# arkCyber/whisper-rust

Hardware: AMD Instinct MI355X
Metric: real-time factor (audio-sec/wall-sec), greedy, 30 s synthetic chunks (higher is better)
Workload: dtype f16 operands / f32 accumulate; 1 GPU; ggml-small-shaped synthetic F16 model, greedy best_of=1 temperature_inc=0, 1 x 30 s 16 kHz f32 chunk per GPU, PCM resident in HBM; flash_attn=False, parallelism=chunk-dp1

## Files before the change

### whisper-rust_amd/csrc/wa_mega.hip

```cpp
#include "wa_device.h"
#include "wa_mega.h"

typedef unsigned long long u64;
#define GAS __attribute__((address_space(1)))
typedef GAS u64 gu64;
typedef GAS unsigned gu32;
typedef const GAS wa_f16 * gch;
typedef const GAS float * gcf;
typedef _Float16 half4v __attribute__((ext_vector_type(4)));
typedef unsigned u32x2 __attribute__((ext_vector_type(2)));
typedef unsigned u32x4 __attribute__((ext_vector_type(4)));

typedef const __attribute__((address_space(4))) wa_mega_args * mg_kargs;
__device__ __forceinline__ mg_kargs mg_uniform(mg_kargs p) {
    const unsigned long long v = (unsigned long long) p;
    const unsigned lo = __builtin_amdgcn_readfirstlane((unsigned) v), hi = __builtin_amdgcn_readfirstlane((unsigned) (v >> 32));
    return (mg_kargs) (((unsigned long long) hi << 32) | lo);
}

#define MG_THREADS 512
#define MG_NW (MG_THREADS / 64)
#define MG_NP3 4
#define MG_SPIN_LIMIT 20000u
#ifndef MG_DEFER
// ... 1054 lines not shown
#pragma unroll
        for (int cc = 0; cc < 32; ++cc) dv[cc] = (cc < 16 ? dbl0 : dbl1)[(cc & 15) * 64 + tid];
        __builtin_amdgcn_sched_barrier(0);
#pragma unroll
        for (int cc = 0; cc < 32; ++cc) sumf += dv[cc];
        if (tslot >= 0) mg_trace(A, tid == 0, tslot + 2, mg_now() + (sumf == 1e300 ? 1u : 0u));
        if constexpr (Q) {
            const float y = (float) sumf;
            float a = fabsf(y);
            a = fmaxf(a, dpp_f32<0x128>(a)); a = fmaxf(a, dpp_f32<0x124>(a)); a = fmaxf(a, dpp_f32<0x122>(a)); a = fmaxf(a, dpp_f32<0x121>(a));
            a = fmaxf(a, __shfl_xor(a, 16, 32));
            const float dsc = a / 127.f, id = a != 0.0f ? 127.f / a : 0.0f;
            const unsigned q = (unsigned) (int) rintf(y * id) & 0xffu;
            const unsigned w = q | (dpp_u32<0x101>(q) << 8) | (dpp_u32<0x102>(q) << 16) | (dpp_u32<0x103>(q) << 24);
            gu64 * eb = edge + (size_t) (2 * h + (tid >> 5)) * 9;
            if ((tid & 3) == 0) gr_store(eb + ((tid & 31) >> 2), seq, w);
            if ((tid & 31) == 0) gr_store(eb + 8, seq, __float_as_uint(h2f(f2h(dsc))));
        } else {
        const unsigned hv = (unsigned) f2h((float) sumf);
        const unsigned hi = dpp_u32<0x101>(hv);
        if ((tid & 1) == 0) gr_store(edge + ((h * 64 + tid) >> 1), seq, (hv & 0xffffu) | (hi << 16));
        }
    }
}

template <bool Q = false>
__device__ __forceinline__ void mg_role_self(mg_kargs A_, int idx_) {
    extern __shared__ __attribute__((aligned(16))) unsigned char smem[];
    const mg_kargs A = mg_uniform(A_);
    const int tid = threadIdx.x, lane = tid & 63;
    const int wave = __builtin_amdgcn_readfirstlane(tid >> 6);
    const int h = __builtin_amdgcn_readfirstlane(idx_);
    mg_ctl c; c.status = (gu32 *) A->status; c.seq = A->seq; c.dead = false;
    mg_chaos_start(c.seq);

    wa_f16 * Ks = (wa_f16 *) smem;
    wa_f16 * Vs = Ks + WA_MEGA_MAX_KV * 64;
    const mg_att_smem M = mg_att_carve(smem + (size_t) WA_MEGA_MAX_KV * 64 * 2 * 2, WA_MEGA_MAX_KV);
    const int d = A->d, n_kv = A->n_kv, kv_head = A->kv_head, L = A->n_layer;
    const int a = tid & 3, kslot = tid >> 2;
    if (wave == 0) mg_pick(A, lane, (int *) (smem + MG_PICK_OFF));
    for (int l = 0; l < L; ++l) {
        {
            const gch kc = (gch) A->kv_k + (size_t) l * A->kv_layer_stride + h * 64;
            const gch vc = (gch) A->kv_v + (size_t) l * A->kv_layer_stride + h * 64;
            const int n16 = n_kv * 8;
            u32x4 tk[8], tv[8];
#pragma unroll
            for (int j = 0; j < 8; ++j) {
                const int idx = tid + MG_THREADS * j;
                if (idx < n16) {
                    tk[j] = *(const GAS u32x4 *) (kc + (size_t) (idx >> 3) * d + (idx & 7) * 8);
                    tv[j] = *(const GAS u32x4 *) (vc + (size_t) (idx >> 3) * d + (idx & 7) * 8);
                }
            }
#pragma unroll
            for (int j = 0; j < 8; ++j) {
                const int idx = tid + MG_THREADS * j;
                if (idx < n16) { *(u32x4 *) (Ks + (size_t) idx * 8) = tk[j]; *(u32x4 *) (Vs + (size_t) idx * 8) = tv[j]; }
            }
        }
        mg_barrier();
        if (wave == 0) {
            unsigned v[2];
            const unsigned sp = mg_sweep<2>(mg_edge(A, l, E_QKV), [&](int k) {
                if (k == 0) return (lane < 32 ? 0 : (d >> 1)) + h * 32 + (lane & 31);
                return lane < 32 ? d + h * 32 + lane : -1; }, c, lane, v, 1000u + l);
            mg_trace(A, h == 0 && lane == 0, (l * 8 + 6) * 8 + 0, mg_now()); mg_trace(A, h == 0 && lane == 0, (l * 8 + 6) * 8 + 1, sp);
            if (lane < 32) { ((unsigned *) M.qs)[lane] = v[0]; ((unsigned *) (Vs + (size_t) kv_head * 64))[lane] = v[1]; }
            else ((unsigned *) (Ks + (size_t) kv_head * 64))[lane - 32] = v[0];
        }
        mg_barrier();
        float lmax = -INFINITY;
        {
            float qa[8], qb[8];
#pragma unroll
            for (int i = 0; i < 8; ++i) { qa[i] = h2f(M.qs[8 * a + i]); qb[i] = h2f(M.qs[32 + 8 * a + i]); }
            for (int c0 = 0; c0 < n_kv; c0 += MG_THREADS / 4) {
                const int cc = c0 + kslot, cl = cc < n_kv ? cc : n_kv - 1;
                const u32x4 ka = *(const u32x4 *) (Ks + (size_t) cl * 64 + 8 * a), kb = *(const u32x4 *) (Ks + (size_t) cl * 64 + 32 + 8 * a);
                const float r = mg_score(ka, kb, qa, qb, 1.0f);
                if (cc < n_kv) { if (a == 0) M.sc[cc] = r; lmax = fmaxf(lmax, r); }
            }
        }
        mg_trace(A, h == 0 && tid == 0, (l * 8 + 6) * 8 + 4, mg_now());
        {
            lmax = wave_max(lmax);
            if (lane == 0) M.red[wave] = lmax;
            mg_barrier();
            float mx = M.red[0];
#pragma unroll
            for (int k = 1; k < MG_NW; ++k) mx = fmaxf(mx, M.red[k]);
            const int n8 = n_kv & ~7, ng = n8 >> 3;
            float e = 0.0f;
            double ps = 0.0;
            if (tid < n_kv) e = tid < n8 ? wa_expf(M.sc[tid] - mx) : wa_expf_libm(M.sc[tid] - mx);
            {
                float t = e + dpp_f32<0x104>(e);
                t = t + dpp_f32<0x102>(t);
                t = t + dpp_f32<0x101>(t);
                if (tid < n8) ps = (tid & 7) == 0 ? (double) t : 0.0;
                else if (tid < n_kv) ps = (double) e;
            }
            ps = wave_sum_d(ps);
            if (lane == 0) M.redd[wave] = ps;
            mg_barrier();
            const double tot = ((M.redd[0] + M.redd[1]) + (M.redd[2] + M.redd[3])) + ((M.redd[4] + M.redd[5]) + (M.redd[6] + M.redd[7]));
            const double delta = (double) (ng + 8 + 16) * 0x1p-53 * tot * 1.000001;
            const float ilo = (float) (1.0 / (tot + delta)), ihi = (float) (1.0 / (tot - delta));
            if (ilo != ihi && tid == 0 && !c.dead) __hip_atomic_store(c.status, (unsigned) WA_MEGA_REDO, __ATOMIC_RELAXED, __HIP_MEMORY_SCOPE_AGENT);
            if (tid < n_kv) M.p16[tid] = f2h(e * ilo);
            mg_barrier();
        }
        mg_trace(A, h == 0 && tid == 0, (l * 8 + 6) * 8 + 5, mg_now());
        MG_CHAOS_ID(1000 + h, 21u, c.seq);
        const int np = n_kv & ~31, nsteps = np >> 5;
        {
            float acc[4] = { 0.0f, 0.0f, 0.0f, 0.0f };
            const int r0 = wave * 4;
            for (int s = 0; s < nsteps; ++s) {
#pragma unroll
                for (int i = 0; i < 4; ++i)
                    acc[i] = fmaf(h2f(Vs[(size_t) (s * 32 + r0 + i) * 64 + lane]), h2f(M.p16[s * 32 + r0 + i]), acc[i]);
            }
#pragma unroll
            for (int i = 0; i < 4; ++i) M.part[(r0 + i) * 64 + lane] = acc[i];
        }
        mg_barrier();
        mg_attn_finish<Q>(M.part, Vs + (size_t) np * 64, M.p16, np, n_kv - np, mg_edge(A, l, E_AO), h, c.seq, tid, (double *) (Ks + WA_MEGA_KV_ROOM * 64),
                          (double *) (Vs + WA_MEGA_KV_ROOM * 64), A, A->dbg && h == 0 && l == MG_WGTRACE_LAYER ? 3004 : -1);
        mg_trace(A, h == 0 && tid == 0, (l * 8 + 6) * 8 + 3, mg_now());
        mg_barrier();
    }
    unsigned pf[96];
    bool have_pf = false;
    float gw[MG_NP3], gb[MG_NP3];
    if (wave >= 1) mg_prefetch_logits<0, Q>(A, pf, have_pf, lane, wave);
    mg_ln_params<MG_NP3>(gw, gb, A->lnf_w, A->lnf_b, A->d, mg_slot(wave, MG_EX_FINAL), lane);
    mg_final<MG_NP3, 0, Q>(A, c, smem, pf, have_pf, gw, gb, lane, wave);
}

#define MG_CSTEPS 48
#define MG_CGR 2048
#define MG_CGR_MAX 0
#define MG_CGR_SUM 8
#define MG_CGR_XCC 16
#define MG_CGR_PART 64
#define MG_CX_XF 32768
#define MG_CX_XIN (MG_CX_XF + WA_MEGA_MAX_D * 4)
#define MG_CX_LNRED (MG_CX_XIN + WA_MEGA_MAX_D * 2)
#define MG_CX_END (MG_CX_LNRED + 256)
#define MG_CX_TRACE 6144

template <bool Q = false, int CQ = -1>
__device__ __forceinline__ void mg_role_cross(mg_kargs A_, int idx_) {
    extern __shared__ __attribute__((aligned(16))) unsigned char smem[];
    const mg_kargs A = mg_uniform(A_);
    int tid = threadIdx.x, lane = tid & 63;
    const int wave = __builtin_amdgcn_readfirstlane(tid >> 6);
    const int H = A->n_head;
    const int ci = __builtin_amdgcn_readfirstlane(idx_);
    const int h = ci >> 2, w = ci & 3;
    mg_ctl c; c.status = (gu32 *) A->status; c.seq = A->seq; c.dead = false;
    mg_chaos_start(c.seq);
    const unsigned seq = c.seq;

    float  * part  = (float *) smem;
    wa_f16 * vleft = (wa_f16 *) (smem + 8192);
    float  * sc    = (float *) (smem + 8192 + 4096);
    wa_f16 * p16   = (wa_f16 *) (smem + 8192 + 4096 + 1536);
    wa_f16 * pleft = (wa_f16 *) (smem + 8192 + 4096 + 1536 + 768);
    wa_f16 * qs    = (wa_f16 *) (smem + 8192 + 4096 + 1536 + 768 + 64);
    double * redd  = (double *) (smem + 8192 + 4096 + 1536 + 768 + 64 + 128);
    float  * red   = (float *) (smem + 8192 + 4096 + 1536 + 768 + 64 + 128 + 64);
    float  * bc    = red + 8;

    const int T = A->T, tpad = A->cross_tpad, L = A->n_layer;
    const float kq_scale = A->kq_scale;
    int a = tid & 3, ks = tid >> 2;
    const int np = T & ~31, nsteps = np >> 5, nl = T - np, n8 = T & ~7, ng = n8 >> 3;
    if (wave == 0) mg_pick(A, lane, (int *) (smem + MG_PICK_OFF));
    if (wave == 0) {
        const unsigned xcc = (unsigned) __builtin_amdgcn_s_getreg(20 | (3 << 11)) & 0xfu;
        gu64 * X0 = (gu64 *) A->cross_gr + (size_t) h * MG_CGR + MG_CGR_XCC;
        if (lane == 0) gr_store(X0 + w, seq, xcc);
        unsigned v[1];
        mg_sweep<1>(X0, [&](int) { return lane < 4 ? lane : -1; }, c, lane, v, 2900u);
        const bool same = lane >= 4 || v[0] == xcc;
        if (lane == 0) bc[2] = __builtin_amdgcn_ballot_w64(same) == ~0ull && !c.dead ? 1.0f : 0.0f;
    }
    mg_barrier();
    const bool local = bc[2] != 0.0f;
    const __attribute__((address_space(4))) wa_mega_layer * Ly = (const __attribute__((address_space(4))) wa_mega_layer *) A->layers;
    float  * xf    = (float *) (smem + MG_CX_XF);
    wa_f16 * xin   = (wa_f16 *) (smem + MG_CX_XIN);
    double * lnred = (double *) (smem + MG_CX_LNRED);
    const int d = A->d;
    for (int l = 0; l < L; ++l) {
        if constexpr (CQ >= 0) {
            unsigned z = threadIdx.x; asm volatile("" : "+v"(z));
            tid = (int) z; lane = tid & 63; a = tid & 3; ks = tid >> 2;
        }
        gu64 * X = (gu64 *) A->cross_gr + ((size_t) l * H + h) * MG_CGR;
        const gch kp = (gch) A->cross_k + (size_t) l * A->cross_layer_stride + (size_t) h * tpad * 64;
        const gch vp = (gch) A->cross_v + (size_t) l * A->cross_layer_stride + (size_t) h * tpad * 64;
        u32x4 ka[3], kb[3];
        unsigned short vv[MG_CSTEPS];
#pragma unroll
        for (int p = 0; p < 3; ++p) {
            const int o = p * 128 + ks, cc = 32 * (o >> 3) + 8 * w + (o & 7);
            if (cc < T) { ka[p] = *(const GAS u32x4 *) (kp + (size_t) cc * 64 + 8 * a); kb[p] = *(const GAS u32x4 *) (kp + (size_t) cc * 64 + 32 + 8 * a); }
        }
#pragma unroll
        for (int s = 0; s < MG_CSTEPS; ++s) if (s < nsteps) vv[s] = *(const GAS unsigned short *) (vp + (size_t) (32 * s + 8 * w + wave) * 64 + lane);
        if (w == 0 && tid < 256) {
            const int row = tid >> 3;
            if (row < nl) *(u32x4 *) (vleft + (size_t) tid * 8) = *(const GAS u32x4 *) (vp + (size_t) (np + row) * 64 + (tid & 7) * 8);
        }
        if constexpr (CQ >= 0) {
            unsigned pf[96];
            float gw[2], gb[2];
            const int row = 64 * h + 8 * wave + (lane >> 3);
            const gch wrow = (gch) Ly[l].cq_w + (size_t) row * d + 4 * (lane & 7);
            mg_pf8<CQ>(pf, wrow, true, d >> 5, 0);
            const float bias = ((gcf) Ly[l].cq_b)[row];
            mg_ln_params<2>(gw, gb, Ly[l].ln2_w, Ly[l].ln2_b, d, mg_slot(wave, 0u), lane);
            mg_trace(A, ci == 0 && lane == 0 && wave == 0, (l * 8 + 7) * 8 + 2, mg_now());
            mg_ln3<2>(A, c, mg_edge(A, l, E_X1), gw, gb, mg_slot(wave, 0u), lane, xf, xin, lnred, 2000u + l,
                      ci == 0 && wave == 0 ? MG_CX_TRACE + l * 8 : -1);
            MG_CHAOS_ID(2000 + ci, 30u, seq);
            float v = mg_dot8<CQ>(pf, wrow, true, d >> 5, xin, lane & 7, true);
            v = v + bias;
            const unsigned hq = (unsigned) f2h(v);
            if ((lane & 7) == 0) qs[8 * wave + (lane >> 3)] = (wa_f16) hq;
            if (A->dbg && w == 0) mg_pub_h2(mg_edge(A, l, E_QC), seq, true, row, hq, lane);
            mg_trace(A, ci == 0 && lane == 0 && wave == 0, (l * 8 + 7) * 8 + 0, mg_now());
            if (A->dbg && l == MG_WGTRACE_LAYER && w == 0) mg_trace(A, tid == 0, 3200 + h, mg_now());
        } else if (wave == 0) {
            unsigned v[1];
            mg_trace(A, ci == 0 && lane == 0, (l * 8 + 7) * 8 + 2, mg_now());
            const unsigned sp = mg_sweep<1>(mg_edge(A, l, E_QC), [&](int) { return lane < 32 ? h * 32 + lane : -1; }, c, lane, v, 2000u + l);
            mg_trace(A, ci == 0 && lane == 0, (l * 8 + 7) * 8 + 0, mg_now()); mg_trace(A, ci == 0 && lane == 0, (l * 8 + 7) * 8 + 1, sp);
            if (A->dbg && l == MG_WGTRACE_LAYER && w == 0) mg_trace(A, lane == 0, 3200 + h, mg_now());
            if (lane < 32) ((unsigned *) qs)[lane] = v[0];
        }
        mg_barrier();
#define MG_CX(k) do { if (A->dbg && l == MG_WGTRACE_LAYER) mg_trace(A, ci == 0 && tid == 0, 3010 + (k), mg_now()); } while (0)
        MG_CX(0);
        MG_CHAOS_ID(2000 + ci, 31u, seq);
        float lmax = -INFINITY;
        {
            float qa[8], qb[8];
#pragma unroll
            for (int i = 0; i < 8; ++i) { qa[i] = h2f(qs[8 * a + i]); qb[i] = h2f(qs[32 + 8 * a + i]); }
#pragma unroll
            for (int p = 0; p < 3; ++p) {
                const int o = p * 128 + ks, cc = 32 * (o >> 3) + 8 * w + (o & 7);
                const float r = mg_score(ka[p], kb[p], qa, qb, kq_scale);
                if (cc < T) { if (a == 0) sc[o] = r; lmax = fmaxf(lmax, r); }
            }
        }
        lmax = wave_max(lmax);
        if (lane == 0) red[wave] = lmax;
        MG_CX(1);
        mg_barrier();
        MG_CX(2);
        if (wave == 0) {
            float m = red[0];
#pragma unroll
            for (int k = 1; k < MG_NW; ++k) m = fmaxf(m, red[k]);
            if (lane == 0) gr_store_l(X + MG_CGR_MAX + w, seq, __float_as_uint(m), local);
            unsigned v[1];
            mg_sweep<1>(X + MG_CGR_MAX, [&](int) { return lane < 4 ? lane : -1; }, c, lane, v, 2100u + l);
            float g = lane < 4 ? __uint_as_float(v[0]) : -INFINITY;
            g = fmaxf(g, dpp_f32<0x4e>(g)); g = fmaxf(g, dpp_f32<0xb1>(g));
            if (lane == 0) bc[0] = g;
            MG_CX(3);
        }
        mg_barrier();
        mg_trace(A, ci == 0 && tid == 0, (l * 8 + 7) * 8 + 4, mg_now());
        const float mx = bc[0];
        {
            double ps = 0.0;
            if (tid < 8 * MG_CSTEPS) {
                const int g = 4 * (tid >> 3) + w, cc = 8 * g + (tid & 7);
                const float e = cc < n8 ? wa_expf(sc[tid] - mx) : (cc < T ? wa_expf_libm(sc[tid] - mx) : 0.0f);
                sc[tid] = e;
                float t = e + dpp_f32<0x104>(e);
                t = t + dpp_f32<0x102>(t);
                t = t + dpp_f32<0x101>(t);
                if (g < ng) ps = (tid & 7) == 0 ? (double) t : 0.0;
                else ps = (double) e;
            }
            ps = wave_sum_d(ps);
            if (lane == 0) redd[wave] = ps;
        }
        MG_CX(4);
        mg_barrier();
        if (wave == 0) {
            const double ps = ((redd[0] + redd[1]) + (redd[2] + redd[3])) + ((redd[4] + redd[5]) + (redd[6] + redd[7]));
            const u64 pb = (u64) __double_as_longlong(ps);
            if (lane == 0) { gr_store_l(X + MG_CGR_SUM + 2 * w, seq, (unsigned) pb, local); gr_store_l(X + MG_CGR_SUM + 2 * w + 1, seq, (unsigned) (pb >> 32), local); }
            unsigned v[1];
            mg_sweep<1>(X + MG_CGR_SUM, [&](int) { return lane < 8 ? lane : -1; }, c, lane, v, 2200u + l);
            double tot = 0.0;
#pragma unroll
            for (int k = 0; k < 4; ++k) {
                const unsigned lo = __builtin_amdgcn_readlane(v[0], 2 * k), hi = __builtin_amdgcn_readlane(v[0], 2 * k + 1);
                tot += __longlong_as_double((long long) (((u64) hi << 32) | lo));
            }
            const double delta = (double) (ng + 8 + 16) * 0x1p-53 * tot * 1.000001;
            const float ilo = (float) (1.0 / (tot + delta)), ihi = (float) (1.0 / (tot - delta));
            if (ilo != ihi && lane == 0 && !c.dead) __hip_atomic_store(c.status, (unsigned) WA_MEGA_REDO, __ATOMIC_RELAXED, __HIP_MEMORY_SCOPE_AGENT);
            if (lane == 0) bc[1] = ilo;
            MG_CX(5);
        }
        mg_barrier();
        mg_trace(A, ci == 0 && tid == 0, (l * 8 + 7) * 8 + 5, mg_now());
        const float inv = bc[1];
        if (tid < 8 * MG_CSTEPS) {
            const int cc = 32 * (tid >> 3) + 8 * w + (tid & 7);
            if (cc < T) {
                const wa_f16 ph = f2h(sc[tid] * inv);
                p16[(tid & 7) * MG_CSTEPS + (tid >> 3)] = ph;
                if (cc >= np) { if (w == 0) pleft[cc - np] = ph; else gr_store_l(X + MG_CGR_PART + (w - 1) * 576 + 512 + (tid & 7), seq, (unsigned) ph, local); }
            }
        }
        mg_barrier();
        MG_CX(6);
        MG_CHAOS_ID(2000 + ci, 32u, seq);
        {
            float acc = 0.0f;
            half8 pw[MG_CSTEPS / 8];
#pragma unroll
            for (int k = 0; k < MG_CSTEPS / 8; ++k) pw[k] = *(const half8 *) (p16 + wave * MG_CSTEPS + 8 * k);
#pragma unroll
            for (int s = 0; s < MG_CSTEPS; ++s) if (s < nsteps) acc = fmaf(h2f(vv[s]), (float) pw[s >> 3][s & 7], acc);
            if (w == 0) part[wave * 64 + lane] = acc;
            else gr_store_l(X + MG_CGR_PART + (w - 1) * 576 + wave * 64 + lane, seq, __float_as_uint(acc), local);
        }
        mg_trace(A, ci == 0 && tid == 0, (l * 8 + 7) * 8 + 6, mg_now());
        if (w == 0) {
            if (wave >= 1 && wave <= 6) {
                const int ww = (wave - 1) >> 1, half = (wave - 1) & 1;
                gu64 * src = X + MG_CGR_PART + ww * 576;
                unsigned v[5];
                mg_sweep<5>(src, [&](int k) { return k < 4 ? half * 256 + 64 * k + lane : (half == 0 && lane < 8 && 8 * (ww + 1) + lane < nl ? 512 + lane : -1); }, c, lane, v, 2300u + l);
#pragma unroll
                for (int k = 0; k < 4; ++k) part[(8 * (ww + 1) + 4 * half + k) * 64 + lane] = __uint_as_float(v[k]);
                if (half == 0 && lane < 8) { const int cc = 8 * (ww + 1) + lane; if (cc < nl) pleft[cc] = (wa_f16) v[4]; }
            }
            mg_barrier();
            mg_trace(A, ci == 0 && tid == 0, (l * 8 + 7) * 8 + 7, mg_now());
            mg_attn_finish<Q>(part, vleft, pleft - np, np, nl, mg_edge(A, l, E_AO2), h, seq, tid, (double *) (smem + 16384), (double *) (smem + 24576), A,
                              A->dbg && ci == 0 && l == MG_WGTRACE_LAYER ? 3000 : -1);
            mg_trace(A, ci == 0 && tid == 0, (l * 8 + 7) * 8 + 3, mg_now());
            if (A->dbg && l == MG_WGTRACE_LAYER) mg_trace(A, tid == 0, 3100 + h, mg_now());
        }
        mg_barrier();
    }
    unsigned pf[96];
    bool have_pf = false;
    float gw[MG_NP3], gb[MG_NP3];
    if (wave >= 1) mg_prefetch_logits<0, Q>(A, pf, have_pf, lane, wave);
    mg_ln_params<MG_NP3>(gw, gb, A->lnf_w, A->lnf_b, A->d, mg_slot(wave, MG_EX_FINAL), lane);
    mg_final<MG_NP3, 0, Q>(A, c, smem, pf, have_pf, gw, gb, lane, wave);
}

#ifndef MG_CQ_TU
__global__ __launch_bounds__(MG_THREADS) void k_decode_mega(const wa_mega_args A) {
    int role, idx;
    mg_role_of((int) gridDim.x, A.n_head, (int) blockIdx.x, role, idx);
    const mg_kargs Ap = (mg_kargs) __builtin_amdgcn_kernarg_segment_ptr();
    if (role == 0) {
        if (A.d == 768) mg_role_gemv<2, 24>(Ap, idx); else if (A.d < 768) mg_role_gemv<2, 0>(Ap, idx);
        else mg_role_gemv<MG_NP3, 0>(Ap, idx);
    }
    else if (role == 1) mg_role_self(Ap, idx);
    else                mg_role_cross(Ap, idx);
}


__global__ __launch_bounds__(MG_THREADS) void k_decode_mega_q(const wa_mega_args A) {
    int role, idx;
    mg_role_of((int) gridDim.x, A.n_head, (int) blockIdx.x, role, idx);
    const mg_kargs Ap = (mg_kargs) __builtin_amdgcn_kernarg_segment_ptr();
    if (role == 0) {
        if (A.d == 768) mg_role_gemv<2, 24, true>(Ap, idx); else if (A.d < 768) mg_role_gemv<2, 0, true>(Ap, idx);
        else if (A.d == 1280) mg_role_gemv<MG_NP3, 40, true>(Ap, idx); else mg_role_gemv<MG_NP3, 0, true>(Ap, idx);
    }
    else if (role == 1) mg_role_self<true>(Ap, idx);
    else                mg_role_cross<true>(Ap, idx);
}

size_t wa_mega_lds_bytes() {
    const size_t s_self  = (size_t) WA_MEGA_MAX_KV * 64 * 2 * 2 + MG_ATT_SMEM(WA_MEGA_MAX_KV);
    const size_t s_cross = MG_CX_END;
    const size_t s_gemv  = MG_PICK_OFF;
    size_t m = s_self > s_cross ? s_self : s_cross;
    m = m > s_gemv ? m : s_gemv;
    if (m > MG_PICK_OFF || (MG_PICK_OFF & 255) != 0) abort();
    return MG_PICK_OFF + MG_PICK_BYTES;
}

bool wa_launch_decode_mega(hipStream_t s, const wa_mega_args & a, int n_wg) {
    static bool attr_set[64] = {};
    const size_t lds = wa_mega_lds_bytes();
    int dev = 0;
    (void) hipGetDevice(&dev);
    if (!attr_set[dev & 63]) {
        if (hipFuncSetAttribute((const void *) k_decode_mega, hipFuncAttributeMaxDynamicSharedMemorySize, (int) lds) != hipSuccess ||
            hipFuncSetAttribute((const void *) k_decode_mega_q, hipFuncAttributeMaxDynamicSharedMemorySize, (int) lds) != hipSuccess) return false;
        attr_set[dev & 63] = true;
    }
    if (MG_DEFER && !a.quant && a.d == 768) return wa_launch_decode_mega_cq(s, a, n_wg, lds);
    if (a.quant) hipLaunchKernelGGL(k_decode_mega_q, dim3(n_wg), dim3(MG_THREADS), lds, s, a);
    else         hipLaunchKernelGGL(k_decode_mega, dim3(n_wg), dim3(MG_THREADS), lds, s, a);
    return hipGetLastError() == hipSuccess;
}
#else
__global__ __launch_bounds__(MG_THREADS) void k_decode_mega_cq(const wa_mega_args A) {
    int role, idx;
    mg_role_of((int) gridDim.x, A.n_head, (int) blockIdx.x, role, idx);
    const mg_kargs Ap = (mg_kargs) __builtin_amdgcn_kernarg_segment_ptr();
    if (role == 0)      mg_role_gemv<2, 24, false, true>(Ap, idx);
    else if (role == 1) mg_role_self(Ap, idx);
    else                mg_role_cross<false, 24>(Ap, idx);
}

bool wa_launch_decode_mega_cq(hipStream_t s, const wa_mega_args & a, int n_wg, size_t lds) {
    static bool attr_set[64] = {};
    int dev = 0;
    (void) hipGetDevice(&dev);
    if (!attr_set[dev & 63]) {
        if (hipFuncSetAttribute((const void *) k_decode_mega_cq, hipFuncAttributeMaxDynamicSharedMemorySize, (int) lds) != hipSuccess) return false;
        attr_set[dev & 63] = true;
    }
    hipLaunchKernelGGL(k_decode_mega_cq, dim3(n_wg), dim3(MG_THREADS), lds, s, a);
    return hipGetLastError() == hipSuccess;
}
#endif
```

Baseline: 351.4 x real-time.

## Split cross-attention work by head dimension instead of by key chunks in CQ role

Adds a dedicated cross-attention role for the deferred d=768 path. Each of the four workgroups per head now owns 16 of the 64 value dimensions and computes scores over all keys locally. This removes the cross-workgroup max, sum and partial-output exchanges through global memory. K/V tiles are staged in LDS, which costs redundant score computation per workgroup and extra LDS traffic. The generic role loses its CQ template path.

```diff
diff --git a/whisper-rust_amd/csrc/wa_mega.hip b/whisper-rust_amd/csrc/wa_mega.hip
--- a/whisper-rust_amd/csrc/wa_mega.hip
+++ b/whisper-rust_amd/csrc/wa_mega.hip
@@ -1230,11 +1230,11 @@
 #define MG_CX_END (MG_CX_LNRED + 256)
 #define MG_CX_TRACE 6144
 
-template <bool Q = false, int CQ = -1>
+template <bool Q = false>
 __device__ __forceinline__ void mg_role_cross(mg_kargs A_, int idx_) {
     extern __shared__ __attribute__((aligned(16))) unsigned char smem[];
     const mg_kargs A = mg_uniform(A_);
-    int tid = threadIdx.x, lane = tid & 63;
+    const int tid = threadIdx.x, lane = tid & 63;
     const int wave = __builtin_amdgcn_readfirstlane(tid >> 6);
     const int H = A->n_head;
     const int ci = __builtin_amdgcn_readfirstlane(idx_);
@@ -1255,7 +1255,7 @@
 
     const int T = A->T, tpad = A->cross_tpad, L = A->n_layer;
     const float kq_scale = A->kq_scale;
-    int a = tid & 3, ks = tid >> 2;
+    const int a = tid & 3, ks = tid >> 2;
     const int np = T & ~31, nsteps = np >> 5, nl = T - np, n8 = T & ~7, ng = n8 >> 3;
     if (wave == 0) mg_pick(A, lane, (int *) (smem + MG_PICK_OFF));
     if (wave == 0) {
@@ -1269,16 +1269,7 @@
     }
     mg_barrier();
     const bool local = bc[2] != 0.0f;
-    const __attribute__((address_space(4))) wa_mega_layer * Ly = (const __attribute__((address_space(4))) wa_mega_layer *) A->layers;
-    float  * xf    = (float *) (smem + MG_CX_XF);
-    wa_f16 * xin   = (wa_f16 *) (smem + MG_CX_XIN);
-    double * lnred = (double *) (smem + MG_CX_LNRED);
-    const int d = A->d;
     for (int l = 0; l < L; ++l) {
-        if constexpr (CQ >= 0) {
-            unsigned z = threadIdx.x; asm volatile("" : "+v"(z));
-            tid = (int) z; lane = tid & 63; a = tid & 3; ks = tid >> 2;
-        }
         gu64 * X = (gu64 *) A->cross_gr + ((size_t) l * H + h) * MG_CGR;
         const gch kp = (gch) A->cross_k + (size_t) l * A->cross_layer_stride + (size_t) h * tpad * 64;
         const gch vp = (gch) A->cross_v + (size_t) l * A->cross_layer_stride + (size_t) h * tpad * 64;
@@ -1295,7 +1286,282 @@
             const int row = tid >> 3;
             if (row < nl) *(u32x4 *) (vleft + (size_t) tid * 8) = *(const GAS u32x4 *) (vp + (size_t) (np + row) * 64 + (tid & 7) * 8);
         }
-        if constexpr (CQ >= 0) {
+        if (wave == 0) {
+            unsigned v[1];
+            mg_trace(A, ci == 0 && lane == 0, (l * 8 + 7) * 8 + 2, mg_now());
+            const unsigned sp = mg_sweep<1>(mg_edge(A, l, E_QC), [&](int) { return lane < 32 ? h * 32 + lane : -1; }, c, lane, v, 2000u + l);
+            mg_trace(A, ci == 0 && lane == 0, (l * 8 + 7) * 8 + 0, mg_now()); mg_trace(A, ci == 0 && lane == 0, (l * 8 + 7) * 8 + 1, sp);
+            if (A->dbg && l == MG_WGTRACE_LAYER && w == 0) mg_trace(A, lane == 0, 3200 + h, mg_now());
+            if (lane < 32) ((unsigned *) qs)[lane] = v[0];
+        }
+        mg_barrier();
+#define MG_CX(k) do { if (A->dbg && l == MG_WGTRACE_LAYER) mg_trace(A, ci == 0 && tid == 0, 3010 + (k), mg_now()); } while (0)
+        MG_CX(0);
+        MG_CHAOS_ID(2000 + ci, 31u, seq);
+        float lmax = -INFINITY;
+        {
+            float qa[8], qb[8];
+#pragma unroll
+            for (int i = 0; i < 8; ++i) { qa[i] = h2f(qs[8 * a + i]); qb[i] = h2f(qs[32 + 8 * a + i]); }
+#pragma unroll
+            for (int p = 0; p < 3; ++p) {
+                const int o = p * 128 + ks, cc = 32 * (o >> 3) + 8 * w + (o & 7);
+                const float r = mg_score(ka[p], kb[p], qa, qb, kq_scale);
+                if (cc < T) { if (a == 0) sc[o] = r; lmax = fmaxf(lmax, r); }
+            }
+        }
+        lmax = wave_max(lmax);
+        if (lane == 0) red[wave] = lmax;
+        MG_CX(1);
+        mg_barrier();
+        MG_CX(2);
+        if (wave == 0) {
+            float m = red[0];
+#pragma unroll
+            for (int k = 1; k < MG_NW; ++k) m = fmaxf(m, red[k]);
+            if (lane == 0) gr_store_l(X + MG_CGR_MAX + w, seq, __float_as_uint(m), local);
+            unsigned v[1];
+            mg_sweep<1>(X + MG_CGR_MAX, [&](int) { return lane < 4 ? lane : -1; }, c, lane, v, 2100u + l);
+            float g = lane < 4 ? __uint_as_float(v[0]) : -INFINITY;
+            g = fmaxf(g, dpp_f32<0x4e>(g)); g = fmaxf(g, dpp_f32<0xb1>(g));
+            if (lane == 0) bc[0] = g;
+            MG_CX(3);
+        }
+        mg_barrier();
+        mg_trace(A, ci == 0 && tid == 0, (l * 8 + 7) * 8 + 4, mg_now());
+        const float mx = bc[0];
+        {
+            double ps = 0.0;
+            if (tid < 8 * MG_CSTEPS) {
+                const int g = 4 * (tid >> 3) + w, cc = 8 * g + (tid & 7);
+                const float e = cc < n8 ? wa_expf(sc[tid] - mx) : (cc < T ? wa_expf_libm(sc[tid] - mx) : 0.0f);
+                sc[tid] = e;
+                float t = e + dpp_f32<0x104>(e);
+                t = t + dpp_f32<0x102>(t);
+                t = t + dpp_f32<0x101>(t);
+                if (g < ng) ps = (tid & 7) == 0 ? (double) t : 0.0;
+                else ps = (double) e;
+            }
+            ps = wave_sum_d(ps);
+            if (lane == 0) redd[wave] = ps;
+        }
+        MG_CX(4);
+        mg_barrier();
+        if (wave == 0) {
+            const double ps = ((redd[0] + redd[1]) + (redd[2] + redd[3])) + ((redd[4] + redd[5]) + (redd[6] + redd[7]));
+            const u64 pb = (u64) __double_as_longlong(ps);
+            if (lane == 0) { gr_store_l(X + MG_CGR_SUM + 2 * w, seq, (unsigned) pb, local); gr_store_l(X + MG_CGR_SUM + 2 * w + 1, seq, (unsigned) (pb >> 32), local); }
+            unsigned v[1];
+            mg_sweep<1>(X + MG_CGR_SUM, [&](int) { return lane < 8 ? lane : -1; }, c, lane, v, 2200u + l);
+            double tot = 0.0;
+#pragma unroll
+            for (int k = 0; k < 4; ++k) {
+                const unsigned lo = __builtin_amdgcn_readlane(v[0], 2 * k), hi = __builtin_amdgcn_readlane(v[0], 2 * k + 1);
+                tot += __longlong_as_double((long long) (((u64) hi << 32) | lo));
+            }
+            const double delta = (double) (ng + 8 + 16) * 0x1p-53 * tot * 1.000001;
+            const float ilo = (float) (1.0 / (tot + delta)), ihi = (float) (1.0 / (tot - delta));
+            if (ilo != ihi && lane == 0 && !c.dead) __hip_atomic_store(c.status, (unsigned) WA_MEGA_REDO, __ATOMIC_RELAXED, __HIP_MEMORY_SCOPE_AGENT);
+            if (lane == 0) bc[1] = ilo;
+            MG_CX(5);
+        }
+        mg_barrier();
+        mg_trace(A, ci == 0 && tid == 0, (l * 8 + 7) * 8 + 5, mg_now());
+        const float inv = bc[1];
+        if (tid < 8 * MG_CSTEPS) {
+            const int cc = 32 * (tid >> 3) + 8 * w + (tid & 7);
+            if (cc < T) {
+                const wa_f16 ph = f2h(sc[tid] * inv);
+                p16[(tid & 7) * MG_CSTEPS + (tid >> 3)] = ph;
+                if (cc >= np) { if (w == 0) pleft[cc - np] = ph; else gr_store_l(X + MG_CGR_PART + (w - 1) * 576 + 512 + (tid & 7), seq, (unsigned) ph, local); }
+            }
+        }
+        mg_barrier();
+        MG_CX(6);
+        MG_CHAOS_ID(2000 + ci, 32u, seq);
+        {
+            float acc = 0.0f;
+            half8 pw[MG_CSTEPS / 8];
+#pragma unroll
+            for (int k = 0; k < MG_CSTEPS / 8; ++k) pw[k] = *(const half8 *) (p16 + wave * MG_CSTEPS + 8 * k);
+#pragma unroll
+            for (int s = 0; s < MG_CSTEPS; ++s) if (s < nsteps) acc = fmaf(h2f(vv[s]), (float) pw[s >> 3][s & 7], acc);
+            if (w == 0) part[wave * 64 + lane] = acc;
+            else gr_store_l(X + MG_CGR_PART + (w - 1) * 576 + wave * 64 + lane, seq, __float_as_uint(acc), local);
+        }
+        mg_trace(A, ci == 0 && tid == 0, (l * 8 + 7) * 8 + 6, mg_now());
+        if (w == 0) {
+            if (wave >= 1 && wave <= 6) {
+                const int ww = (wave - 1) >> 1, half = (wave - 1) & 1;
+                gu64 * src = X + MG_CGR_PART + ww * 576;
+                unsigned v[5];
+                mg_sweep<5>(src, [&](int k) { return k < 4 ? half * 256 + 64 * k + lane : (half == 0 && lane < 8 && 8 * (ww + 1) + lane < nl ? 512 + lane : -1); }, c, lane, v, 2300u + l);
+#pragma unroll
+                for (int k = 0; k < 4; ++k) part[(8 * (ww + 1) + 4 * half + k) * 64 + lane] = __uint_as_float(v[k]);
+                if (half == 0 && lane < 8) { const int cc = 8 * (ww + 1) + lane; if (cc < nl) pleft[cc] = (wa_f16) v[4]; }
+            }
+            mg_barrier();
+            mg_trace(A, ci == 0 && tid == 0, (l * 8 + 7) * 8 + 7, mg_now());
+            mg_attn_finish<Q>(part, vleft, pleft - np, np, nl, mg_edge(A, l, E_AO2), h, seq, tid, (double *) (smem + 16384), (double *) (smem + 24576), A,
+                              A->dbg && ci == 0 && l == MG_WGTRACE_LAYER ? 3000 : -1);
+            mg_trace(A, ci == 0 && tid == 0, (l * 8 + 7) * 8 + 3, mg_now());
+            if (A->dbg && l == MG_WGTRACE_LAYER) mg_trace(A, tid == 0, 3100 + h, mg_now());
+        }
+        mg_barrier();
+    }
+    unsigned pf[96];
+    bool have_pf = false;
+    float gw[MG_NP3], gb[MG_NP3];
+    if (wave >= 1) mg_prefetch_logits<0, Q>(A, pf, have_pf, lane, wave);
+    mg_ln_params<MG_NP3>(gw, gb, A->lnf_w, A->lnf_b, A->d, mg_slot(wave, MG_EX_FINAL), lane);
+    mg_final<MG_NP3, 0, Q>(A, c, smem, pf, have_pf, gw, gb, lane, wave);
+}
+
+#ifndef MG_CQ_TU
+__global__ __launch_bounds__(MG_THREADS) void k_decode_mega(const wa_mega_args A) {
+    int role, idx;
+    mg_role_of((int) gridDim.x, A.n_head, (int) blockIdx.x, role, idx);
+    const mg_kargs Ap = (mg_kargs) __builtin_amdgcn_kernarg_segment_ptr();
+    if (role == 0) {
+        if (A.d == 768) mg_role_gemv<2, 24>(Ap, idx); else if (A.d < 768) mg_role_gemv<2, 0>(Ap, idx);
+        else mg_role_gemv<MG_NP3, 0>(Ap, idx);
+    }
+    else if (role == 1) mg_role_self(Ap, idx);
+    else                mg_role_cross(Ap, idx);
+}
+
+
+__global__ __launch_bounds__(MG_THREADS) void k_decode_mega_q(const wa_mega_args A) {
+    int role, idx;
+    mg_role_of((int) gridDim.x, A.n_head, (int) blockIdx.x, role, idx);
+    const mg_kargs Ap = (mg_kargs) __builtin_amdgcn_kernarg_segment_ptr();
+    if (role == 0) {
+        if (A.d == 768) mg_role_gemv<2, 24, true>(Ap, idx); else if (A.d < 768) mg_role_gemv<2, 0, true>(Ap, idx);
+        else if (A.d == 1280) mg_role_gemv<MG_NP3, 40, true>(Ap, idx); else mg_role_gemv<MG_NP3, 0, true>(Ap, idx);
+    }
+    else if (role == 1) mg_role_self<true>(Ap, idx);
+    else                mg_role_cross<true>(Ap, idx);
+}
+
+size_t wa_mega_lds_bytes() {
+    const size_t s_self  = (size_t) WA_MEGA_MAX_KV * 64 * 2 * 2 + MG_ATT_SMEM(WA_MEGA_MAX_KV);
+    const size_t s_cross = MG_CX_END;
+    const size_t s_gemv  = MG_PICK_OFF;
+    size_t m = s_self > s_cross ? s_self : s_cross;
+    m = m > s_gemv ? m : s_gemv;
+    if (m > MG_PICK_OFF || (MG_PICK_OFF & 255) != 0) abort();
+    return MG_PICK_OFF + MG_PICK_BYTES;
+}
+
+bool wa_launch_decode_mega(hipStream_t s, const wa_mega_args & a, int n_wg) {
+    static bool attr_set[64] = {};
+    const size_t lds = wa_mega_lds_bytes();
+    int dev = 0;
+    (void) hipGetDevice(&dev);
+    if (!attr_set[dev & 63]) {
+        if (hipFuncSetAttribute((const void *) k_decode_mega, hipFuncAttributeMaxDynamicSharedMemorySize, (int) lds) != hipSuccess ||
+            hipFuncSetAttribute((const void *) k_decode_mega_q, hipFuncAttributeMaxDynamicSharedMemorySize, (int) lds) != hipSuccess) return false;
+        attr_set[dev & 63] = true;
+    }
+    if (MG_DEFER && !a.quant && a.d == 768) return wa_launch_decode_mega_cq(s, a, n_wg, lds);
+    if (a.quant) hipLaunchKernelGGL(k_decode_mega_q, dim3(n_wg), dim3(MG_THREADS), lds, s, a);
+    else         hipLaunchKernelGGL(k_decode_mega, dim3(n_wg), dim3(MG_THREADS), lds, s, a);
+    return hipGetLastError() == hipSuccess;
+}
+#else
+#define MG_CY_PART 0
+#define MG_CY_DBL  2048
+#define MG_CY_PT   6144
+#define MG_CY_QS   9216
+#define MG_CY_REDD 9344
+#define MG_CY_RED  9408
+#define MG_CY_V    MG_CX_END
+#define MG_CY_K    (MG_CY_V + (MG_CSTEPS / 8) * MG_THREADS * 16)
+#define MG_CY_END  (MG_CY_K + 8 * MG_THREADS * 16)
+static_assert(MG_CY_RED + 32 <= MG_CX_XF && (MG_CY_V & 15) == 0 && MG_CY_END <= MG_PICK_OFF, "LDS of the d = 768 cross-attention role");
+static_assert(3 * MG_THREADS >= WA_MEGA_MAX_T && MG_CSTEPS * 32 >= WA_MEGA_MAX_T && MG_THREADS == 32 * 16, "three cells per thread; thread = (chain, dimension)");
+
+__device__ __forceinline__ float mg_wave_max(float v) {
+    v = fmaxf(v, dpp_f32<0x128>(v)); v = fmaxf(v, dpp_f32<0x124>(v)); v = fmaxf(v, dpp_f32<0x122>(v)); v = fmaxf(v, dpp_f32<0x121>(v));
+    const int b = __builtin_bit_cast(int, v);
+    const float r0 = __builtin_bit_cast(float, __builtin_amdgcn_readlane(b, 0)), r1 = __builtin_bit_cast(float, __builtin_amdgcn_readlane(b, 16));
+    const float r2 = __builtin_bit_cast(float, __builtin_amdgcn_readlane(b, 32)), r3 = __builtin_bit_cast(float, __builtin_amdgcn_readlane(b, 48));
+    return fmaxf(fmaxf(r0, r1), fmaxf(r2, r3));
+}
+
+template <int CQ>
+__device__ __forceinline__ void mg_role_cross_cq(mg_kargs A_, int idx_) {
+    extern __shared__ __attribute__((aligned(16))) unsigned char smem[];
+    const mg_kargs A = mg_uniform(A_);
+    int tid = threadIdx.x, lane = tid & 63;
+    const int wave = __builtin_amdgcn_readfirstlane(tid >> 6);
+    const int ci = __builtin_amdgcn_readfirstlane(idx_);
+    const int h = ci >> 2, w = ci & 3;
+    mg_ctl c; c.status = (gu32 *) A->status; c.seq = A->seq; c.dead = false;
+    mg_chaos_start(c.seq);
+    const unsigned seq = c.seq;
+
+    float  * part  = (float *) (smem + MG_CY_PART);
+    double * dbl   = (double *) (smem + MG_CY_DBL);
+    wa_f16 * pT    = (wa_f16 *) (smem + MG_CY_PT);
+    wa_f16 * qs    = (wa_f16 *) (smem + MG_CY_QS);
+    double * redd  = (double *) (smem + MG_CY_REDD);
+    float  * red   = (float *) (smem + MG_CY_RED);
+    u32x4  * vl    = (u32x4 *) (smem + MG_CY_V);
+    u32x4  * kl    = (u32x4 *) (smem + MG_CY_K);
+    float  * xf    = (float *) (smem + MG_CX_XF);
+    wa_f16 * xin   = (wa_f16 *) (smem + MG_CX_XIN);
+    double * lnred = (double *) (smem + MG_CX_LNRED);
+
+    const int T = A->T, tpad = A->cross_tpad, L = A->n_layer, d = A->d;
+    const float kq_scale = A->kq_scale;
+    const int np = T & ~31, nsteps = np >> 5, nl = T - np, n8 = T & ~7, ng = n8 >> 3;
+    if (wave == 0) mg_pick(A, lane, (int *) (smem + MG_PICK_OFF));
+    const __attribute__((address_space(4))) wa_mega_layer * Ly = (const __attribute__((address_space(4))) wa_mega_layer *) A->layers;
+    for (int l = 0; l < L; ++l) {
+        {
+            unsigned z = threadIdx.x; asm volatile("" : "+v"(z));
+            tid = (int) z; lane = tid & 63;
+        }
+        const gch kp = (gch) A->cross_k + (size_t) l * A->cross_layer_stride + (size_t) h * tpad * 64;
+        const gch vp = (gch) A->cross_v + (size_t) l * A->cross_layer_stride + (size_t) h * tpad * 64 + 16 * w;
+        {
+            unsigned short vv[MG_CSTEPS];
+            const gch vt = vp + (size_t) (tid >> 4) * 64 + (tid & 15);
+#pragma unroll
+            for (int s = 0; s < MG_CSTEPS; ++s) vv[s] = s < nsteps ? *(const GAS unsigned short *) (vt + (size_t) s * (32 * 64)) : (unsigned short) 0;
+            const int c2 = 2 * MG_THREADS + tid;
+            u32x4 k2[8];
+            if (c2 < T) {
+#pragma unroll
+                for (int i = 0; i < 8; ++i) k2[i] = *(const GAS u32x4 *) (kp + (size_t) c2 * 64 + 8 * i);
+            }
+#pragma unroll
+            for (int k = 0; k < MG_CSTEPS / 8; ++k) {
+                if (8 * k < nsteps) {
+                    u32x4 pk;
+                    pk.x = (unsigned) vv[8 * k + 0] | ((unsigned) vv[8 * k + 1] << 16); pk.y = (unsigned) vv[8 * k + 2] | ((unsigned) vv[8 * k + 3] << 16);
+                    pk.z = (unsigned) vv[8 * k + 4] | ((unsigned) vv[8 * k + 5] << 16); pk.w = (unsigned) vv[8 * k + 6] | ((unsigned) vv[8 * k + 7] << 16);
+                    vl[k * MG_THREADS + tid] = pk;
+                }
+            }
+            if (c2 < T) {
+#pragma unroll
+                for (int i = 0; i < 8; ++i) kl[i * MG_THREADS + tid] = k2[i];
+            }
+        }
+        u32x4 kr[2][8];
+#pragma unroll
+        for (int p = 0; p < 2; ++p) {
+            const int cc = MG_THREADS * p + tid;
+            if (cc < T) {
+#pragma unroll
+                for (int i = 0; i < 8; ++i) kr[p][i] = *(const GAS u32x4 *) (kp + (size_t) cc * 64 + 8 * i);
+            }
+        }
+        unsigned short vleft = 0;
+        if ((tid >> 4) < nl) vleft = *(const GAS unsigned short *) (vp + (size_t) (np + (tid >> 4)) * 64 + (tid & 15));
+        {
             unsigned pf[96];
             float gw[2], gb[2];
             const int row = 64 * h + 8 * wave + (lane >> 3);
@@ -1314,196 +1580,132 @@
             if (A->dbg && w == 0) mg_pub_h2(mg_edge(A, l, E_QC), seq, true, row, hq, lane);
             mg_trace(A, ci == 0 && lane == 0 && wave == 0, (l * 8 + 7) * 8 + 0, mg_now());
             if (A->dbg && l == MG_WGTRACE_LAYER && w == 0) mg_trace(A, tid == 0, 3200 + h, mg_now());
-        } else if (wave == 0) {
-            unsigned v[1];
-            mg_trace(A, ci == 0 && lane == 0, (l * 8 + 7) * 8 + 2, mg_now());
-            const unsigned sp = mg_sweep<1>(mg_edge(A, l, E_QC), [&](int) { return lane < 32 ? h * 32 + lane : -1; }, c, lane, v, 2000u + l);
-            mg_trace(A, ci == 0 && lane == 0, (l * 8 + 7) * 8 + 0, mg_now()); mg_trace(A, ci == 0 && lane == 0, (l * 8 + 7) * 8 + 1, sp);
-            if (A->dbg && l == MG_WGTRACE_LAYER && w == 0) mg_trace(A, lane == 0, 3200 + h, mg_now());
-            if (lane < 32) ((unsigned *) qs)[lane] = v[0];
-        }
-        mg_barrier();
-#define MG_CX(k) do { if (A->dbg && l == MG_WGTRACE_LAYER) mg_trace(A, ci == 0 && tid == 0, 3010 + (k), mg_now()); } while (0)
-        MG_CX(0);
+        }
+        mg_barrier();
+#define MG_CY(k) do { if (A->dbg && l == MG_WGTRACE_LAYER) mg_trace(A, ci == 0 && tid == 0, 3010 + (k), mg_now()); } while (0)
+        MG_CY(0);
         MG_CHAOS_ID(2000 + ci, 31u, seq);
+        float sv[3] = { 0.0f, 0.0f, 0.0f };
         float lmax = -INFINITY;
         {
-            float qa[8], qb[8];
-#pragma unroll
-            for (int i = 0; i < 8; ++i) { qa[i] = h2f(qs[8 * a + i]); qb[i] = h2f(qs[32 + 8 * a + i]); }
+            half8 q8[8];
+#pragma unroll
+            for (int i = 0; i < 8; ++i) q8[i] = *(const half8 *) (qs + 8 * i);
 #pragma unroll
             for (int p = 0; p < 3; ++p) {
-                const int o = p * 128 + ks, cc = 32 * (o >> 3) + 8 * w + (o & 7);
-                const float r = mg_score(ka[p], kb[p], qa, qb, kq_scale);
-                if (cc < T) { if (a == 0) sc[o] = r; lmax = fmaxf(lmax, r); }
-            }
-        }
-        lmax = wave_max(lmax);
+                if (p < 2 || T > 2 * MG_THREADS) {
+                    half8 k8[8];
+#pragma unroll
+                    for (int i = 0; i < 8; ++i) k8[i] = __builtin_bit_cast(half8, p < 2 ? kr[p < 2 ? p : 0][i] : kl[i * MG_THREADS + tid]);
+                    float s32[32];
+#pragma unroll
+                    for (int j = 0; j < 32; ++j) {
+                        const float t = fmaf((float) k8[j >> 3][j & 7], (float) q8[j >> 3][j & 7], 0.0f);
+                        s32[j] = fmaf((float) k8[4 + (j >> 3)][j & 7], (float) q8[4 + (j >> 3)][j & 7], t);
+                    }
+                    sv[p] = wa_tree32(s32) * kq_scale;
+                    if (MG_THREADS * p + tid < T) lmax = fmaxf(lmax, sv[p]);
+                }
+            }
+        }
+        lmax = mg_wave_max(lmax);
         if (lane == 0) red[wave] = lmax;
-        MG_CX(1);
-        mg_barrier();
-        MG_CX(2);
-        if (wave == 0) {
-            float m = red[0];
-#pragma unroll
-            for (int k = 1; k < MG_NW; ++k) m = fmaxf(m, red[k]);
-            if (lane == 0) gr_store_l(X + MG_CGR_MAX + w, seq, __float_as_uint(m), local);
-            unsigned v[1];
-            mg_sweep<1>(X + MG_CGR_MAX, [&](int) { return lane < 4 ? lane : -1; }, c, lane, v, 2100u + l);
-            float g = lane < 4 ? __uint_as_float(v[0]) : -INFINITY;
-            g = fmaxf(g, dpp_f32<0x4e>(g)); g = fmaxf(g, dpp_f32<0xb1>(g));
-            if (lane == 0) bc[0] = g;
-            MG_CX(3);
-        }
-        mg_barrier();
+        MG_CY(1);
+        mg_barrier();
+        MG_CY(2);
         mg_trace(A, ci == 0 && tid == 0, (l * 8 + 7) * 8 + 4, mg_now());
-        const float mx = bc[0];
+        float mx = red[0];
+#pragma unroll
+        for (int k = 1; k < MG_NW; ++k) mx = fmaxf(mx, red[k]);
+        float e[3];
         {
             double ps = 0.0;
-            if (tid < 8 * MG_CSTEPS) {
-                const int g = 4 * (tid >> 3) + w, cc = 8 * g + (tid & 7);
-                const float e = cc < n8 ? wa_expf(sc[tid] - mx) : (cc < T ? wa_expf_libm(sc[tid] - mx) : 0.0f);
-                sc[tid] = e;
-                float t = e + dpp_f32<0x104>(e);
+#pragma unroll
+            for (int p = 0; p < 3; ++p) {
+                const int cc = MG_THREADS * p + tid;
+                e[p] = cc < n8 ? wa_expf(sv[p] - mx) : (cc < T ? wa_expf_libm(sv[p] - mx) : 0.0f);
+                float t = e[p] + dpp_f32<0x104>(e[p]);
                 t = t + dpp_f32<0x102>(t);
                 t = t + dpp_f32<0x101>(t);
-                if (g < ng) ps = (tid & 7) == 0 ? (double) t : 0.0;
-                else ps = (double) e;
+                const double pp = cc < n8 ? ((tid & 7) == 0 ? (double) t : 0.0) : (double) e[p];
+                ps = p == 0 ? pp : ps + pp;
             }
             ps = wave_sum_d(ps);
             if (lane == 0) redd[wave] = ps;
         }
-        MG_CX(4);
-        mg_barrier();
-        if (wave == 0) {
-            const double ps = ((redd[0] + redd[1]) + (redd[2] + redd[3])) + ((redd[4] + redd[5]) + (redd[6] + redd[7]));
-            const u64 pb = (u64) __double_as_longlong(ps);
-            if (lane == 0) { gr_store_l(X + MG_CGR_SUM + 2 * w, seq, (unsigned) pb, local); gr_store_l(X + MG_CGR_SUM + 2 * w + 1, seq, (unsigned) (pb >> 32), local); }
-            unsigned v[1];
-            mg_sweep<1>(X + MG_CGR_SUM, [&](int) { return lane < 8 ? lane : -1; }, c, lane, v, 2200u + l);
-            double tot = 0.0;
-#pragma unroll
-            for (int k = 0; k < 4; ++k) {
-                const unsigned lo = __builtin_amdgcn_readlane(v[0], 2 * k), hi = __builtin_amdgcn_readlane(v[0], 2 * k + 1);
-                tot += __longlong_as_double((long long) (((u64) hi << 32) | lo));
-            }
+        MG_CY(3);
+        mg_barrier();
+        {
+            const double tot = ((redd[0] + redd[1]) + (redd[2] + redd[3])) + ((redd[4] + redd[5]) + (redd[6] + redd[7]));
             const double delta = (double) (ng + 8 + 16) * 0x1p-53 * tot * 1.000001;
             const float ilo = (float) (1.0 / (tot + delta)), ihi = (float) (1.0 / (tot - delta));
-            if (ilo != ihi && lane == 0 && !c.dead) __hip_atomic_store(c.status, (unsigned) WA_MEGA_REDO, __ATOMIC_RELAXED, __HIP_MEMORY_SCOPE_AGENT);
-            if (lane == 0) bc[1] = ilo;
-            MG_CX(5);
+            if (ilo != ihi && tid == 0 && !c.dead) __hip_atomic_store(c.status, (unsigned) WA_MEGA_REDO, __ATOMIC_RELAXED, __HIP_MEMORY_SCOPE_AGENT);
+            MG_CY(4);
+#pragma unroll
+            for (int p = 0; p < 3; ++p) {
+                const int cc = MG_THREADS * p + tid;
+                if (cc < T) pT[(cc & 31) * MG_CSTEPS + (cc >> 5)] = f2h(e[p] * ilo);
+            }
         }
         mg_barrier();
         mg_trace(A, ci == 0 && tid == 0, (l * 8 + 7) * 8 + 5, mg_now());
-        const float inv = bc[1];
-        if (tid < 8 * MG_CSTEPS) {
-            const int cc = 32 * (tid >> 3) + 8 * w + (tid & 7);
-            if (cc < T) {
-                const wa_f16 ph = f2h(sc[tid] * inv);
-                p16[(tid & 7) * MG_CSTEPS + (tid >> 3)] = ph;
-                if (cc >= np) { if (w == 0) pleft[cc - np] = ph; else gr_store_l(X + MG_CGR_PART + (w - 1) * 576 + 512 + (tid & 7), seq, (unsigned) ph, local); }
-            }
-        }
-        mg_barrier();
-        MG_CX(6);
+        MG_CY(5);
         MG_CHAOS_ID(2000 + ci, 32u, seq);
         {
+            const int r = tid >> 4;
+            half8 pw[MG_CSTEPS / 8], vw[MG_CSTEPS / 8];
+#pragma unroll
+            for (int k = 0; k < MG_CSTEPS / 8; ++k) { pw[k] = *(const half8 *) (pT + r * MG_CSTEPS + 8 * k); vw[k] = __builtin_bit_cast(half8, vl[k * MG_THREADS + tid]); }
             float acc = 0.0f;
-            half8 pw[MG_CSTEPS / 8];
-#pragma unroll
-            for (int k = 0; k < MG_CSTEPS / 8; ++k) pw[k] = *(const half8 *) (p16 + wave * MG_CSTEPS + 8 * k);
-#pragma unroll
-            for (int s = 0; s < MG_CSTEPS; ++s) if (s < nsteps) acc = fmaf(h2f(vv[s]), (float) pw[s >> 3][s & 7], acc);
-            if (w == 0) part[wave * 64 + lane] = acc;
-            else gr_store_l(X + MG_CGR_PART + (w - 1) * 576 + wave * 64 + lane, seq, __float_as_uint(acc), local);
+#pragma unroll
+            for (int s = 0; s < MG_CSTEPS; ++s) if (s < nsteps) acc = fmaf((float) vw[s >> 3][s & 7], (float) pw[s >> 3][s & 7], acc);
+            part[tid] = acc;
+            float nzero = -0.0f;
+            asm volatile("" : "+v"(nzero));
+            const float pr = fmaf(h2f(vleft), h2f(pT[r * MG_CSTEPS + nsteps]), nzero);
+            dbl[tid] = (double) (r < nl ? pr : -0.0f);
         }
         mg_trace(A, ci == 0 && tid == 0, (l * 8 + 7) * 8 + 6, mg_now());
-        if (w == 0) {
-            if (wave >= 1 && wave <= 6) {
-                const int ww = (wave - 1) >> 1, half = (wave - 1) & 1;
-                gu64 * src = X + MG_CGR_PART + ww * 576;
-                unsigned v[5];
-                mg_sweep<5>(src, [&](int k) { return k < 4 ? half * 256 + 64 * k + lane : (half == 0 && lane < 8 && 8 * (ww + 1) + lane < nl ? 512 + lane : -1); }, c, lane, v, 2300u + l);
-#pragma unroll
-                for (int k = 0; k < 4; ++k) part[(8 * (ww + 1) + 4 * half + k) * 64 + lane] = __uint_as_float(v[k]);
-                if (half == 0 && lane < 8) { const int cc = 8 * (ww + 1) + lane; if (cc < nl) pleft[cc] = (wa_f16) v[4]; }
-            }
-            mg_barrier();
-            mg_trace(A, ci == 0 && tid == 0, (l * 8 + 7) * 8 + 7, mg_now());
-            mg_attn_finish<Q>(part, vleft, pleft - np, np, nl, mg_edge(A, l, E_AO2), h, seq, tid, (double *) (smem + 16384), (double *) (smem + 24576), A,
-                              A->dbg && ci == 0 && l == MG_WGTRACE_LAYER ? 3000 : -1);
-            mg_trace(A, ci == 0 && tid == 0, (l * 8 + 7) * 8 + 3, mg_now());
-            if (A->dbg && l == MG_WGTRACE_LAYER) mg_trace(A, tid == 0, 3100 + h, mg_now());
-        }
-        mg_barrier();
+        mg_barrier();
+        mg_trace(A, ci == 0 && tid == 0, (l * 8 + 7) * 8 + 7, mg_now());
+        MG_CY(6);
+        if (tid < 16) {
+            const int ts = A->dbg && ci == 0 && l == MG_WGTRACE_LAYER ? 3000 : -1;
+            if (ts >= 0) mg_trace(A, tid == 0, ts, mg_now());
+            float s32[32];
+            double dv[32];
+#pragma unroll
+            for (int r = 0; r < 32; ++r) { s32[r] = part[r * 16 + tid]; dv[r] = dbl[r * 16 + tid]; }
+            __builtin_amdgcn_sched_barrier(0);
+            double sumf = (double) wa_tree32(s32);
+            if (ts >= 0) mg_trace(A, tid == 0, ts + 1, mg_now() + (sumf == 1e300 ? 1u : 0u));
+#pragma unroll
+            for (int cc = 0; cc < 32; ++cc) sumf += dv[cc];
+            if (ts >= 0) mg_trace(A, tid == 0, ts + 2, mg_now() + (sumf == 1e300 ? 1u : 0u));
+            const unsigned hv = (unsigned) f2h((float) sumf);
+            const unsigned hi = dpp_u32<0x101>(hv);
+            if ((tid & 1) == 0) gr_store(mg_edge(A, l, E_AO2) + ((h * 64 + 16 * w + tid) >> 1), seq, (hv & 0xffffu) | (hi << 16));
+        }
+        mg_trace(A, ci == 0 && tid == 0, (l * 8 + 7) * 8 + 3, mg_now());
+        if (A->dbg && l == MG_WGTRACE_LAYER && w == 0) mg_trace(A, tid == 0, 3100 + h, mg_now());
+        mg_barrier();
+#undef MG_CY
     }
     unsigned pf[96];
     bool have_pf = false;
     float gw[MG_NP3], gb[MG_NP3];
-    if (wave >= 1) mg_prefetch_logits<0, Q>(A, pf, have_pf, lane, wave);
+    if (wave >= 1) mg_prefetch_logits<0, false>(A, pf, have_pf, lane, wave);
     mg_ln_params<MG_NP3>(gw, gb, A->lnf_w, A->lnf_b, A->d, mg_slot(wave, MG_EX_FINAL), lane);
-    mg_final<MG_NP3, 0, Q>(A, c, smem, pf, have_pf, gw, gb, lane, wave);
-}
-
-#ifndef MG_CQ_TU
-__global__ __launch_bounds__(MG_THREADS) void k_decode_mega(const wa_mega_args A) {
-    int role, idx;
-    mg_role_of((int) gridDim.x, A.n_head, (int) blockIdx.x, role, idx);
-    const mg_kargs Ap = (mg_kargs) __builtin_amdgcn_kernarg_segment_ptr();
-    if (role == 0) {
-        if (A.d == 768) mg_role_gemv<2, 24>(Ap, idx); else if (A.d < 768) mg_role_gemv<2, 0>(Ap, idx);
-        else mg_role_gemv<MG_NP3, 0>(Ap, idx);
-    }
-    else if (role == 1) mg_role_self(Ap, idx);
-    else                mg_role_cross(Ap, idx);
-}
-
-
-__global__ __launch_bounds__(MG_THREADS) void k_decode_mega_q(const wa_mega_args A) {
-    int role, idx;
-    mg_role_of((int) gridDim.x, A.n_head, (int) blockIdx.x, role, idx);
-    const mg_kargs Ap = (mg_kargs) __builtin_amdgcn_kernarg_segment_ptr();
-    if (role == 0) {
-        if (A.d == 768) mg_role_gemv<2, 24, true>(Ap, idx); else if (A.d < 768) mg_role_gemv<2, 0, true>(Ap, idx);
-        else if (A.d == 1280) mg_role_gemv<MG_NP3, 40, true>(Ap, idx); else mg_role_gemv<MG_NP3, 0, true>(Ap, idx);
-    }
-    else if (role == 1) mg_role_self<true>(Ap, idx);
-    else                mg_role_cross<true>(Ap, idx);
-}
-
-size_t wa_mega_lds_bytes() {
-    const size_t s_self  = (size_t) WA_MEGA_MAX_KV * 64 * 2 * 2 + MG_ATT_SMEM(WA_MEGA_MAX_KV);
-    const size_t s_cross = MG_CX_END;
-    const size_t s_gemv  = MG_PICK_OFF;
-    size_t m = s_self > s_cross ? s_self : s_cross;
-    m = m > s_gemv ? m : s_gemv;
-    if (m > MG_PICK_OFF || (MG_PICK_OFF & 255) != 0) abort();
-    return MG_PICK_OFF + MG_PICK_BYTES;
-}
-
-bool wa_launch_decode_mega(hipStream_t s, const wa_mega_args & a, int n_wg) {
-    static bool attr_set[64] = {};
-    const size_t lds = wa_mega_lds_bytes();
-    int dev = 0;
-    (void) hipGetDevice(&dev);
-    if (!attr_set[dev & 63]) {
-        if (hipFuncSetAttribute((const void *) k_decode_mega, hipFuncAttributeMaxDynamicSharedMemorySize, (int) lds) != hipSuccess ||
-            hipFuncSetAttribute((const void *) k_decode_mega_q, hipFuncAttributeMaxDynamicSharedMemorySize, (int) lds) != hipSuccess) return false;
-        attr_set[dev & 63] = true;
-    }
-    if (MG_DEFER && !a.quant && a.d == 768) return wa_launch_decode_mega_cq(s, a, n_wg, lds);
-    if (a.quant) hipLaunchKernelGGL(k_decode_mega_q, dim3(n_wg), dim3(MG_THREADS), lds, s, a);
-    else         hipLaunchKernelGGL(k_decode_mega, dim3(n_wg), dim3(MG_THREADS), lds, s, a);
-    return hipGetLastError() == hipSuccess;
-}
-#else
+    mg_final<MG_NP3, 0, false>(A, c, smem, pf, have_pf, gw, gb, lane, wave);
+}
+
 __global__ __launch_bounds__(MG_THREADS) void k_decode_mega_cq(const wa_mega_args A) {
     int role, idx;
     mg_role_of((int) gridDim.x, A.n_head, (int) blockIdx.x, role, idx);
     const mg_kargs Ap = (mg_kargs) __builtin_amdgcn_kernarg_segment_ptr();
     if (role == 0)      mg_role_gemv<2, 24, false, true>(Ap, idx);
     else if (role == 1) mg_role_self(Ap, idx);
-    else                mg_role_cross<false, 24>(Ap, idx);
+    else                mg_role_cross_cq<24>(Ap, idx);
 }
 
 bool wa_launch_decode_mega_cq(hipStream_t s, const wa_mega_args & a, int n_wg, size_t lds) {
```

New measurement: 354.0 x real-time, median of 6. No clear change (+0.7%).
